# crockwell/far

Hardware: AMD Instinct MI355X
Metric: image-pairs/sec (match+solve+regress) at 640x480 (higher is better)
Workload: dtype f32

## Files before the change

### far_amd/_lib.py

```python
import ctypes
import os

from . import flags

_HERE = os.path.dirname(os.path.abspath(__file__))
LIB_PATH = flags.value('FAR_HIP_LIB') or os.path.join(_HERE, 'lib', 'libfar_hip.so')

c_p = ctypes.c_void_p
c_i = ctypes.c_int
c_f = ctypes.c_float
c_d = ctypes.c_double
c_sz = ctypes.c_size_t
c_l = ctypes.c_long
c_u32 = ctypes.c_uint32

SIGNATURES = {
    'far_abi_version': (c_i, []),
    'far_last_hip_error': (c_i, []),
    'far_set_tuning': (c_i, [c_i, c_i]),
    'far_mfma_probe_f16': (c_i, [c_i, c_i, c_i, c_p, c_p, c_p]),
    'far_dual_softmax_workspace_bytes': (c_sz, [c_i, c_i, c_i]),
    'far_dual_softmax_stats_f32': (c_i, [c_p, c_p, c_i, c_i, c_i, c_i, c_f, c_f, c_f, c_p, c_p, c_p, c_p, c_p, c_p]),
    'far_coarse_match_f32': (c_i, [c_p, c_p, c_i, c_i, c_i, c_i, c_f, c_f, c_i, c_i, c_i, c_i, c_i, c_f,
                                   c_p, c_p, c_p, c_p, c_p, c_p, c_p, c_p, c_p, c_p, c_p, c_p, c_p, c_p, c_p, c_p]),
# ... 48 lines not shown
    'far_bn_train_stats_f32': (c_i, [c_p, c_l, c_i, c_p, c_p, c_f, c_f, c_p, c_p, c_p, c_p, c_p, c_p, c_p, c_l, c_p]),
    'far_bn_train_bwd_f32': (c_i, [c_p, c_p, c_p, c_p, c_p, c_p, c_l, c_i, c_i, c_f, c_p, c_p, c_p, c_p, c_p, c_l, c_p]),
    'far_conv_packed_bytes': (c_sz, [c_i, c_i, c_i, c_i, c_i]),
    'far_conv_pack_f32': (c_i, [c_p, c_i, c_i, c_i, c_i, c_i, c_i, c_p, c_p]),
    'far_weight_scale_f32': (c_i, [c_p, c_l, c_p, c_p]),
    'far_conv_pack_view_f32': (c_i, [c_p, c_l, c_l, c_l, c_i, c_i, c_i, c_i, c_i, c_p, c_p, c_p]),
    'far_enc_layer_saved_floats': (c_l, [c_p]),
    'far_enc_layer_grads_floats': (c_l, [c_p]),
    'far_enc_layer_fwd_ws_bytes': (c_l, [c_p]),
    'far_enc_layer_bwd_ws_bytes': (c_l, [c_p]),
    'far_enc_layer_grads_offsets': (c_i, [c_p, c_p]),
    'far_enc_layer_fwd': (c_i, [c_p, c_p, c_p, c_p, c_p, c_p, c_l, c_p]),
    'far_enc_layer_bwd': (c_i, [c_p, c_p, c_p, c_p, c_p, c_p, c_p, c_l, c_p]),
    'far_stream_fork': (c_p, [c_p, c_i]),
    'far_stream_join': (c_i, [c_p, c_i]),
    'far_pack_table_bytes': (c_l, [c_i]),
    'far_pack_table_build': (c_i, [c_p, c_i, c_p, c_p]),
    'far_pack_table_run': (c_i, [c_p, c_i, c_p]),
    'far_conv_pack_view_scaled_f32': (c_i, [c_p, c_l, c_l, c_l, c_i, c_i, c_i, c_i, c_i, c_p, c_p, c_p, c_p, c_p]),
    'far_conv_pack_auto_f32': (c_i, [c_p, c_i, c_i, c_i, c_i, c_i, c_p, c_p, c_p]),
    'far_grad_scale_f32': (c_i, [c_p, c_l, c_p, c_p]),
    'far_conv_nhwc_f32': (c_i, [c_p, c_p]),
    'far_linear_kv_workspace_bytes': (c_sz, [c_l, c_i]),
    'far_linear_kv_image_bytes': (c_sz, [c_l]),
    'far_linear_kv_f16s': (c_i, [c_p, c_i, c_p, c_p, c_p, c_p]),
    'far_linear_q_apply_f16s': (c_i, [c_p, c_i, c_i, c_p, c_f, c_p]),
    'far_linear_gather_f16s': (c_i, [c_p, c_p, c_p, c_i, c_i, c_i, c_l, c_i, c_i, c_p]),
    'far_wino_packed_bytes': (c_sz, [c_i, c_i]),
    'far_wino_pack_view_scaled_f32': (c_i, [c_p, c_l, c_l, c_l, c_i, c_i, c_p, c_p, c_p, c_p, c_p]),
    'far_conv3x3_wino_f32': (c_i, [c_p, c_p]),
    'far_emm_pv_f16s_workspace_bytes': (c_sz, [c_i, c_i]),
    'far_emm_pv_f16s': (c_i, [c_p, c_p, c_p, c_p, c_i, c_i, c_i, c_f, c_i, c_l, c_l, c_i, c_p, c_p, c_p, c_p]),
    'far_emm_pv_f16': (c_i, [c_p, c_p, c_p, c_p, c_i, c_i, c_i, c_f, c_i, c_l, c_l, c_i, c_p, c_p, c_p, c_p]),
    'far_emm_pv_f16s_copy_stats': (c_i, [c_p, c_i, c_i, c_p, c_p, c_p]),
    'far_emm_bwd_workspace_bytes': (c_sz, [c_i, c_i]),
    'far_emm_bwd_f16': (c_i, [c_p, c_p, c_p, c_p, c_p, c_p, c_p, c_p, c_i, c_i, c_f, c_p, c_p, c_p, c_p]),
    'far_corr_volume_warp_workspace_bytes': (c_sz, [c_i, c_i]),
    'far_corr_volume_warp_f32': (c_i, [c_p, c_p, c_p, c_i, c_i, c_i, c_p, c_p, c_p]),
    'far_conv_wgrad_ws_bytes': (c_l, [c_i, c_i, c_i, c_i, c_i, c_i, c_i]),
    'far_conv_wgrad_f16s': (c_i, [c_p, c_p, c_i, c_i, c_i, c_i, c_i, c_i, c_i, c_i, c_p, c_p, c_l, c_p, c_p, c_p]),
    'far_stem7x7_nhwc_f32': (c_i, [c_p, c_p, c_p, c_p, c_i, c_i, c_i, c_i, c_p, c_p]),
    'far_stem7x7_wgrad_ws_bytes': (c_l, [c_i, c_i, c_i, c_i]),
    'far_stem7x7_wgrad_f32': (c_i, [c_p, c_p, c_i, c_i, c_i, c_i, c_p, c_l, c_p, c_p]),
    'far_pose_pack_f64': (c_i, [c_p] * 8 + [c_i] + [c_p] * 6 + [c_p]),
    'far_pose_features_f32': (c_i, [c_p, c_i, c_p, c_i, c_p, c_i, c_p, c_i, c_p, c_i, c_p, c_p, c_p]),
    'far_rows_linear_packed_bytes': (c_sz, [c_i, c_i]),
    'far_rows_linear_workspace_bytes': (c_sz, [c_i, c_i, c_i]),
    'far_rows_linear_pack_f32': (c_i, [c_p, c_i, c_i, c_p, c_p]),
    'far_rows_linear_f32': (c_i, [c_p, c_l, c_p, c_p, c_p, c_l, c_i, c_i, c_i, c_i, c_p, c_l, c_p, c_p]),
    'far_emm_contract_workspace_bytes': (c_sz, [c_i]),
    'far_emm_contract_f32': (c_i, [c_p, c_i, c_l, c_l, c_p, c_p, c_i, c_i, c_p, c_p, c_p]),
    'far_solver_workspace_bytes': (c_sz, [c_i, c_i, c_i, c_i]),
    'far_solver_f64': (c_i, [c_p, c_p, c_p, c_i, c_i, c_i, c_p, c_p, c_p, c_i, c_p, c_p, c_i, c_d, c_i, c_i, c_u32, c_p]
                       + [c_p] * 14 + [c_p, c_p]),
    'far_ransac_f64': (c_i, [c_p, c_p, c_p, c_i, c_i, c_i, c_p, c_p, c_p, c_i, c_d, c_i, c_i, c_u32, c_p] + [c_p] * 6 + [c_p, c_p]),
    'far_eightpoint_f64': (c_i, [c_p, c_p, c_p, c_i, c_i, c_p, c_p]),
    'far_decompose_essential_f64': (c_i, [c_p, c_l, c_p, c_p, c_p, c_p]),
    'far_build_id': (ctypes.c_char_p, []),
}



class ConvDesc(ctypes.Structure):
    _fields_ = [(n, ctypes.c_void_p) for n in ('x', 'x2', 'packed', 'scale', 'shift', 'res', 'ln_gamma', 'ln_beta',
                                               'post_res', 'up', 'y')] + \
               [('N', ctypes.c_long)] + \
# ... 68 lines not shown
```

### far_amd/csrc/emm_bilinear_f16s.hip

```cpp
#include "common.h"
#include <type_traits>

typedef float f32x4v __attribute__((ext_vector_type(4)));

namespace {

typedef _Float16 f16x8 __attribute__((ext_vector_type(8)));
typedef __attribute__((address_space(1))) const void* gptr_t;
typedef __attribute__((address_space(3))) void* lptr_t;

constexpr int D = 64;
constexpr int DV = 70;
constexpr int DVP = 96;
constexpr int KT = 64;
constexpr int CREF_ROW = 80;
constexpr float QK_PRESCALE = 16.0f;
constexpr float V_PRESCALE = 64.0f;
constexpr float NEG_HUGE = -1.0e30f;
constexpr int PAD_REF = 1 << 24;
constexpr int ROW_REF0 = -(1 << 24);

struct ZLayout {
    int heads, P, rot;
    long head_stride, prob_stride;
    __device__ __forceinline__ size_t base(long z) const {
        const long pz = z / heads;
        const int hh = (int)(z - pz * heads);
        return (size_t)hh * head_stride + (size_t)((pz + rot) % P) * prob_stride;
    }
};

__device__ __forceinline__ void split1(float x, _Float16& hi, _Float16& lo) {
    hi = (_Float16)x;
    lo = (_Float16)(x - (float)hi);
}

__global__ void k_prep_qk(const float* __restrict__ x, ZLayout lay, int Z, int N, int Np, _Float16* __restrict__ hi, _Float16* __restrict__ lo,
                          int* __restrict__ overflow) {
    const long total = (long)Z * Np * 8;
    bool bad = false;
    for (long t = (long)blockIdx.x * blockDim.x + threadIdx.x; t < total; t += (long)gridDim.x * blockDim.x) {
        const int slot = (int)(t & 7);
        const long row = t >> 3;
        const int i = (int)(row % Np);
        const long z = row / Np;
        f16x8 vh, vl;
        if (i < N) {
            const float* src = x + lay.base(z) + (size_t)i * D + slot * 8;
// ... 177 lines not shown

__global__ __launch_bounds__(256) void k_prep_v(const float* __restrict__ v, ZLayout lay, const float* __restrict__ pos,
                                               const float2* __restrict__ colstat, int Z, int N, int Np,
                                               _Float16* __restrict__ oh, _Float16* __restrict__ ol,
                                               int* __restrict__ cref) {
    __shared__ float tile[KT][DV + 3];
    const int ntile = Np / KT;
    const int z = blockIdx.x / ntile, jt = blockIdx.x - z * ntile;
    const int tid = threadIdx.x;
    for (int i = tid; i < KT * DV; i += 256) {
        const int r = i / DV, c = i - r * DV;
        const int j = jt * KT + r;
        float x = 0.f;
        if (j < N) {
            x = c < D ? v[lay.base(z) + (size_t)j * D + c] : pos[(size_t)j * 6 + (c - D)];
            const float2 cs = colstat[(size_t)z * N + j];
            x = x / (cs.y * __builtin_amdgcn_exp2f(cs.x - ceilf(cs.x))) * V_PRESCALE;
        }
        tile[r][c] = x;
    }
    if (tid < KT) {
        const int j = jt * KT + tid;
        cref[(size_t)z * Np + j] = j < N ? (int)ceilf(fminf(fmaxf(colstat[(size_t)z * N + j].x, -1.0e6f), 1.0e6f)) : PAD_REF;
    }
    __syncthreads();
    const size_t base = ((size_t)z * ntile + jt) * DVP * KT;
    for (int i = tid; i < DVP * 8; i += 256) {
        const int b = i >> 3, slot = i & 7;
        const int ct = slot >> 2, g = slot & 3;
        f16x8 vh, vl;
#pragma unroll
        for (int e = 0; e < 8; ++e) {
            const int key = 32 * ct + 16 * (g >> 1) + 4 * (g & 1) + (e < 4 ? e : e + 4);
            const float x = b < DV ? tile[key][b] : 0.f;
            _Float16 hh, ll;
            split1(x, hh, ll);
            vh[e] = hh; vl[e] = ll;
        }
        const size_t o = base + (size_t)b * KT + ((slot ^ ((b >> 1) & 7)) * 8);
        *reinterpret_cast<f16x8*>(oh + o) = vh;
        *reinterpret_cast<f16x8*>(ol + o) = vl;
    }
    __syncthreads();
    if (tid < KT) reinterpret_cast<int*>(oh + base + (size_t)CREF_ROW * KT)[tid] = cref[(size_t)z * Np + jt * KT + tid];
}

constexpr int VT_PLANE = DVP * 128;
constexpr int PV_STAGE = 2 * CT_PLANE + 2 * VT_PLANE;
template <bool MASKED>
__device__ __forceinline__ float tile_rowmax(const f32x16 (&acc)[2], float c1, int j0, int N, int h) {
    float tm = NEG_HUGE;
#pragma unroll
    for (int ct = 0; ct < 2; ++ct)
#pragma unroll
        for (int r = 0; r < 16; ++r) {
            const bool pad = MASKED && j0 + 32 * ct + mfma32_row(r, h) >= N;
            tm = fmaxf(tm, pad ? NEG_HUGE : acc[ct][r]);
        }
    return tm * c1;
}

template <bool SPLIT>
__global__ __launch_bounds__(256, 2) void k_pv(const _Float16* __restrict__ qh, const _Float16* __restrict__ ql,
                                               const _Float16* __restrict__ kh, const _Float16* __restrict__ kl,
                                               const _Float16* __restrict__ vh, const _Float16* __restrict__ vl,
                                               const int* __restrict__ cref, int Z, int N, int Np, float c1,
                                               float2* __restrict__ rowstat, float* __restrict__ T) {
    extern __shared__ __attribute__((aligned(16))) unsigned char lds_all[];
    const int tid = threadIdx.x, wave = tid >> 6, lane = tid & 63, l31 = lane & 31, h = lane >> 5;
    int z, Ib;
    tile_coords(Np / 128, Z, z, Ib);
    const int i0 = Ib * 128 + 32 * wave;
    const int irow = i0 + l31;
    RowFrags rf;
    rf.load(qh, ql, (size_t)z * Np + irow, irow, h);
    rf.arrived();

    f32x16 tacc[3];
#pragma unroll
    for (int bt = 0; bt < 3; ++bt)
#pragma unroll
        for (int r = 0; r < 16; ++r) tacc[bt][r] = 0.f;
    int R = ROW_REF0;
    float sum = 0.f, comp = 0.f;

    const int ntile = Np / KT;
    const unsigned char* vsrc_h = reinterpret_cast<const unsigned char*>(vh + (size_t)z * ntile * DVP * KT) + tid * 16;
    const unsigned char* vsrc_l = reinterpret_cast<const unsigned char*>(vl + (size_t)z * ntile * DVP * KT) + tid * 16;
    auto request = [&](int jt) {
        unsigned char* const st = lds_all + (jt & 1) * PV_STAGE;
        dma_col_tile_async(st, kh, kl, (size_t)z * Np + jt * KT, tid, wave);
        const unsigned dv = lds_addr_uniform(st + 2 * CT_PLANE + wave * 1024);
#pragma unroll
        for (int j = 0; j < 3; ++j) {
            glds16(vsrc_h + (size_t)jt * VT_PLANE + j * 4096, dv + j * 4096);
            glds16(vsrc_l + (size_t)jt * VT_PLANE + j * 4096, dv + VT_PLANE + j * 4096);
        }
    };
    request(0);
    for (int jt = 0; jt < ntile; ++jt) {
// ... 32 lines not shown
#pragma unroll
        for (int ct = 0; ct < 2; ++ct) {
#pragma unroll
            for (int u = 0; u < 2; ++u) {
                f16x8 ph, pl;
                const int4 cA = *reinterpret_cast<const int4*>(lcr + 32 * ct + 16 * u + 4 * h);
                const int4 cB = *reinterpret_cast<const int4*>(lcr + 32 * ct + 16 * u + 8 + 4 * h);
                const int cmv[8] = {cA.x, cA.y, cA.z, cA.w, cB.x, cB.y, cB.z, cB.w};
#pragma unroll
                for (int e = 0; e < 8; e += 2) {
                    const int r = 8 * u + e;
                    const f32x2 x2 = __builtin_elementwise_fma(f32x2{acc[ct][r], acc[ct][r + 1]}, f32x2{c1, c1}, f32x2{nR, nR});
                    float e0 = __builtin_amdgcn_exp2f(x2.x);
                    float e1 = __builtin_amdgcn_exp2f(x2.y);
                    if (RAGGED) {
                        if (jt * KT + 32 * ct + mfma32_row(r, h) >= N) e0 = 0.f;
                        if (jt * KT + 32 * ct + mfma32_row(r + 1, h) >= N) e1 = 0.f;
                    }
                    t2 += f32x2{e0, e1};
                    const f32x2 p2 = f32x2{e0, e1} * f32x2{ldexpf(e0, R - cmv[e] + 15), ldexpf(e1, R - cmv[e + 1] + 15)};
                    f16x2 h2, l2;
                    if (SPLIT) split2(p2, h2, l2);
                    else { h2 = __builtin_convertvector(p2, f16x2); l2 = h2; }
                    ph[e] = h2.x; ph[e + 1] = h2.y;
                    pl[e] = l2.x; pl[e + 1] = l2.y;
                }
                const int slot = 4 * ct + 2 * u + h;
#pragma unroll
                for (int bt = 0; bt < 3; ++bt) {
                    const int b = 32 * bt + l31;
                    const int off = b * 128 + ((slot ^ ((b >> 1) & 7)) * 16);
                    const f16x8 bh = *reinterpret_cast<const f16x8*>(ldv + off);
                    tacc[bt] = __builtin_amdgcn_mfma_f32_32x32x16_f16(ph, bh, tacc[bt], 0, 0, 0);
                    if (SPLIT) {
                        const f16x8 bl = *reinterpret_cast<const f16x8*>(ldv + VT_PLANE + off);
                        tacc[bt] = __builtin_amdgcn_mfma_f32_32x32x16_f16(ph, bl, tacc[bt], 0, 0, 0);
                        tacc[bt] = __builtin_amdgcn_mfma_f32_32x32x16_f16(pl, bh, tacc[bt], 0, 0, 0);
                    }
                }
            }
        }
        };
        if (ragged) pv_tile(std::true_type{});
        else pv_tile(std::false_type{});
        const float y = (t2.x + t2.y) - comp;
        const float ns = sum + y;
        comp = (ns - sum) - y;
        sum = ns;
    }
    sum -= comp;
    const float rsum = sum + shfl_xor_f(sum, 32);
    if (h == 0 && irow < N) rowstat[(size_t)z * N + irow] = make_float2((float)R, rsum);
    const float oscale = (3.0517578125e-05f / V_PRESCALE) / rsum;
#pragma unroll
    for (int bt = 0; bt < 3; ++bt) {
        const int b = 32 * bt + l31;
#pragma unroll
        for (int r = 0; r < 16; ++r) {
            const int rr = mfma32_row(r, h);
            const float sc = __shfl(oscale, rr, 64);
            const int i = i0 + rr;
            if (b < DV && i < N) T[((size_t)z * N + i) * DV + b] = tacc[bt][r] * sc;
        }
    }
}

inline size_t align256(size_t x) { return (x + 255) & ~(size_t)255; }
struct EmmWs {
    _Float16 *qh, *ql, *kh, *kl, *vh, *vl;
    float2 *rowstat, *colstat;
    int* cref;
    size_t bytes;
};
inline EmmWs carve(void* base, int Z, int N) {
    const int Np = (N + 127) / 128 * 128;
    unsigned char* p = (unsigned char*)base;
    size_t o = 0;
    auto take = [&](size_t n) { unsigned char* r = p ? p + o : nullptr; o += align256(n); return r; };
    EmmWs w;
    const size_t qk = (size_t)Z * Np * D * 2, vt = (size_t)Z * (Np / KT) * DVP * KT * 2, st = (size_t)Z * N * 8;
    w.qh = (_Float16*)take(qk); w.ql = (_Float16*)take(qk); w.kh = (_Float16*)take(qk); w.kl = (_Float16*)take(qk);
    w.vh = (_Float16*)take(vt); w.vl = (_Float16*)take(vt);
    w.rowstat = (float2*)take(st); w.colstat = (float2*)take(st);
    w.cref = (int*)take((size_t)Z * Np * 4);
    w.bytes = o;
    return w;
}

}

extern "C" {

size_t far_emm_pv_f16s_workspace_bytes(int Z, int N) {
    if (Z <= 0 || N <= 0) return 0;
    return carve(nullptr, Z, N).bytes;
}

}

template <bool SPLIT>
static int emm_pv_launch(const float* q, const float* k, const float* v, const float* pos, int Z, int N, int Dh, float scale,
                         int heads, long head_stride, long prob_stride, int q_rot, void* ws, float* T_out, int* overflow,
                         hipStream_t stream) {
    far_clear_errors();
    if (!q || !k || !v || !pos || !ws || !T_out || Z <= 0 || N <= 0 || Dh != D || heads < 1 || Z % heads || q_rot < 0 ||
        q_rot >= Z / heads)
        return FAR_EINVAL;
    const ZLayout lay{heads, Z / heads, 0, head_stride, prob_stride};
    const ZLayout layq{heads, Z / heads, q_rot, head_stride, prob_stride};
    const int Np = (N + 127) / 128 * 128;
    const EmmWs w = carve(ws, Z, N);
    const float c1 = scale * 1.44269504088896341f / (QK_PRESCALE * QK_PRESCALE);
    const unsigned gprep = (unsigned)(((long)Z * Np * 8 + 255) / 256 < 65536L * 4 ? ((long)Z * Np * 8 + 255) / 256 : 65536L * 4);
    hipLaunchKernelGGL(k_prep_qk, dim3(gprep), dim3(256), 0, stream, q, layq, Z, N, Np, w.qh, w.ql, overflow);
    hipLaunchKernelGGL(k_prep_qk, dim3(gprep), dim3(256), 0, stream, k, lay, Z, N, Np, w.kh, w.kl, overflow);
    const dim3 grid((unsigned)(Np / 128) * Z);
    const dim3 gstat((unsigned)(Np / 128) * Z);
    hipLaunchKernelGGL(k_rowstats<SPLIT>, gstat, dim3(256), 0, stream, w.kh, w.kl, w.qh, w.ql, Z, N, Np, c1, w.colstat);
    hipLaunchKernelGGL(k_prep_v, dim3((unsigned)(Np / KT) * Z), dim3(256), 0, stream, v, lay, pos, w.colstat, Z, N, Np, w.vh, w.vl, w.cref);
    bool cfg_failed = false;
    FAR_ONCE_PER_DEVICE(cfg_failed = hipFuncSetAttribute((const void*)k_pv<SPLIT>, hipFuncAttributeMaxDynamicSharedMemorySize, 2 * PV_STAGE) != hipSuccess);
    if (cfg_failed) return far_check_launch();
    hipLaunchKernelGGL(k_pv<SPLIT>, grid, dim3(256), 2 * PV_STAGE, stream, w.qh, w.ql, w.kh, w.kl, w.vh, w.vl, w.cref, Z, N, Np, c1,
                       w.rowstat, T_out);
    return far_check_launch();
}

extern "C" {

int far_emm_pv_f16s(const float* q, const float* k, const float* v, const float* pos, int Z, int N, int Dh, float scale,
                    int heads, long head_stride, long prob_stride, int q_rot, void* ws, float* T_out, int* overflow,
                    hipStream_t stream) {
    return emm_pv_launch<true>(q, k, v, pos, Z, N, Dh, scale, heads, head_stride, prob_stride, q_rot, ws, T_out, overflow, stream);
}

int far_emm_pv_f16(const float* q, const float* k, const float* v, const float* pos, int Z, int N, int Dh, float scale,
                   int heads, long head_stride, long prob_stride, int q_rot, void* ws, float* T_out, int* overflow,
                   hipStream_t stream) {
    return emm_pv_launch<false>(q, k, v, pos, Z, N, Dh, scale, heads, head_stride, prob_stride, q_rot, ws, T_out, overflow, stream);
}

int far_emm_pv_f16s_copy_stats(const void* ws, int Z, int N, float* rowstat_out, float* colstat_out, hipStream_t stream) {
    far_clear_errors();
    if (!ws || !rowstat_out || !colstat_out || Z <= 0 || N <= 0) return FAR_EINVAL;
    const EmmWs w = carve(const_cast<void*>(ws), Z, N);
    hipMemcpyAsync(rowstat_out, w.rowstat, (size_t)Z * N * 8, hipMemcpyDeviceToDevice, stream);
    hipMemcpyAsync(colstat_out, w.colstat, (size_t)Z * N * 8, hipMemcpyDeviceToDevice, stream);
    return far_check_launch();
}

}
```

### far_amd/flags.py

```python
import os
from collections import namedtuple

Switch = namedtuple('Switch', 'env module attr off_value neutral scope doc')
SWITCHES = [
    Switch('FAR_NO_WINO', 'far_amd.ops', 'USE_WINO', False, 'parity', 'inference',
           'stride-1 3x3 convolutions on K9 (direct implicit GEMM) instead of K17 (Winograd F(2x2,3x3)); same operator, other summation'),
    Switch('FAR_NO_PAD', 'far_amd.loftr.backbone', 'PAD_CHANNELS', False, 'bitwise', 'inference',
           'the 196-channel backbone maps stored with 196 channels instead of 208 (zero weights for the extra ones: exact zeros)'),
    Switch('FAR_NO_PREFETCH', 'far_amd.loftr.model:LoFTR', 'head_prefetch', False, 'bitwise', 'inference',
           "the head's feature stage computed inside forward_rt_prediction instead of enqueued behind K1"),
    Switch('FAR_NO_SIDE_STREAM', 'far_amd.loftr.model:LoFTR', 'head_side_stream', False, 'bitwise', 'inference',
           "the head's feature stage on the step's own stream behind K1 (rounds 2-5) instead of on a second stream next to K1 and the fine level"),
    Switch('FAR_FPN_STREAM', 'far_amd.loftr.model:LoFTR', 'fpn_side_stream', True, 'bitwise', 'inference',
           "OPT-IN (1 switches it ON; default off): the FPN's fine branch on a side stream next to the coarse transformer and K1 (-0.6 ms per 32 "
           "pairs; off by default because the roofline launch -- K17 208 -> 208 @ 240x320 -- then shares the GPU and its in-step duration "
           "in a kernel trace is no longer its own)"),
    Switch('FAR_NO_GATHER_FUSE', 'far_amd.loftr.stages:FinePreprocess', 'fused_gather', False, 'bitwise', 'inference',
           'FinePreprocess.merge_feat on a materialised window tensor (K3 gather + K9) instead of K9 reading through the match indices'),
    Switch('FAR_NO_KV', 'far_amd.loftr.transformer:LoFTREncoderLayer', 'fused_kv', False, 'parity', 'inference',
           "k, v projections + K5's first half as separate launches instead of K9's k|v epilogue (the K'^T V sum changes order)"),
    Switch('FAR_NO_QAPPLY', 'far_amd.loftr.transformer:LoFTREncoderLayer', 'fused_apply', False, 'parity', 'inference',
           "q projection + K5's second half as separate launches instead of K9's attention-apply epilogue (q no longer stays in split operands)"),
    Switch('FAR_NO_STACK', 'far_amd.loftr.transformer:LocalFeatureTransformer', 'stack_self', False, 'bitwise', 'inference',
           "the two 'self' calls of an encoder layer on the two images separately instead of one call on both"),
    Switch('FAR_NO_BN', 'far_amd.ops', 'USE_HIP_BATCHNORM_TRAIN', False, 'parity', 'training',
           'training-mode BatchNorm on nn.BatchNorm2d + torch activations instead of K19 (tests/test_train_kernels_gpu.py holds K19 to the module)'),
]

ENV_ONLY = {
    'FAR_HIP_LIB': ('load', 'path of another build of libfar_hip.so (tools/ab_build.py: same-box A/B against a git revision); skips the build-id check'),
    'FAR_TUNING': ('load', 'comma-separated key=value pairs handed to far_set_tuning at load time, e.g. FAR_TUNING="10=1,8=1" (keys below)'),
    'FAR_SKIP_ASM_CHECK': ('build', "1: far_amd/build.py does not scan the generated code (K9's asm pixel loads; the LDS-DMA ring rule of every kernel with global_load_lds; the half-register writes of the asm fp16 split) after recompiling"),
    'FAR_EXTRA_HIPCC_FLAGS': ('build', 'extra hipcc flags of an experiment build (-DFAR_WINO_EXP=..., tools/wino_exp.sh); part of the build id'),
    'FAR_COMMIT': ('tools', 'commit stamp tools/collect_profiles.sh / tools/step_floors.py write into the profile files'),
    'FAR_C3_PY_NODE': ('bench', "bench.py --workload c3: the encoder layer's autograd node driven from Python instead of far_enc_layer_fwd / _bwd"),
    'FAR_C3_NO_OVERLAP': ('bench', 'bench.py --workload c3: the layer node without side streams'),
    'FAR_C3_PER_OP': ('bench', 'bench.py --workload c3: one autograd node per operator instead of per layer'),
    'FAR_TORCH_ADAMW': ('bench', 'bench.py --workload c3: torch.optim.AdamW instead of K20'),
    'FAR_CUDNN_BENCHMARK': ('bench', 'bench.py: torch.backends.cudnn.benchmark for the vendor comparison legs'),
}

Tuning = namedtuple('Tuning', 'key default values neutral doc')
TUNING = [
    Tuning(0, 3, (0, 1, 2, 4, 7), 'bitwise', 'bit mask of exact-f32 kernels that stagger wave-slot priorities: 1 k_stats, 2 k_match, 4 k_emm_pv'),
    Tuning(1, 0, (1,), 'parity', 'K1 exact-f32 variant: the other tile shape (another summation order of the row statistics)'),
    Tuning(2, 0, (1,), 'bitwise', 'conf_matrix writer variant A (store pattern)'),
    Tuning(3, 0, (1,), 'bitwise', 'conf_matrix writer variant B (store pattern)'),
    Tuning(4, 0, (1,), 'bitwise', 'K9 without the seven-tile mode / K5 windows on the generic path'),
    Tuning(5, 0, (1, 2, 4), 'bitwise', 'K5 apply: tiles per unit'),
    Tuning(6, 0, (64, 256), 'parity', "K5: tokens per K'^T V chunk (another partial-sum grouping)"),
    Tuning(7, 0, (1,), 'bitwise', 'K9 Linear launches always on full-height tiles'),
    Tuning(8, 0, (1,), 'bitwise', 'K17 splits its operands with the five-instruction split2 instead of v_fma_mix (same values)'),
    Tuning(9, 0, (1,), 'bitwise', 'K17 runs a short last channel block on the full body'),
    Tuning(10, 0, (1,), 'bitwise', "K1's match pass without the tile prescreen"),
    Tuning(11, 0, (1, 2), 'bitwise', "K14's pipeline: 0 = 4 waves / 3 slots / counted waits, two workgroups per CU; 1 = 8 waves / 4 slots / counted, one per CU (round 5's form); 2 = 4 waves / 3 slots / vmcnt(0) per phase (fallback without a wait table)"),
    Tuning(12, 0, (1,), 'parity', "K10's inference form on the exact-f32 matrix instruction instead of split fp16"),
    Tuning(15, 0, (1,), 'bitwise', 'K17: 1 = the multiplying wave group does NOT raise its issue priority (the round-4 kernel)'),
    Tuning(13, 0, (1,), 'bitwise', "K9's FPN-merge epilogue in its generic form everywhere"),
]


def off(env):
    if env not in {s.env for s in SWITCHES}:
        raise KeyError(f'{env} is not a registered far_amd switch (far_amd/flags.py)')
    return os.environ.get(env, '0') not in ('', '0')


def value(env, default=None):
    if env not in ENV_ONLY:
        raise KeyError(f'{env} is not a registered far_amd environment variable (far_amd/flags.py)')
    return os.environ.get(env, default)


def known():
    return {s.env for s in SWITCHES} | set(ENV_ONLY)


def unknown_in_environment():
    skip = ('FAR_WINO_', 'FAR_K9_')
    return sorted(k for k in os.environ if k.startswith('FAR_') and k not in known() and not k.startswith(skip))


def target(sw):
    import importlib
    mod, _, cls = sw.module.partition(':')
    obj = importlib.import_module(mod)
    return (getattr(obj, cls) if cls else obj), sw.attr
```

### far_amd/loftr/transformer.py

```python
import copy
import os
from functools import partial

import torch
import torch.nn as nn

from .. import _vendor as ag
from .. import flags, ops
from ..pose6d import pose_mean_6d, pose_std_6d


class LinearAttention(nn.Module):

    def __init__(self, eps=1e-6, use_num_corres=False):
        super().__init__()
        self.eps = eps
        self.use_num_corres = use_num_corres

    def forward(self, queries, keys, values, q_mask=None, kv_mask=None, loftr_preds=None):
        N, L, H, D = queries.shape
        S = keys.shape[1]
        if ag.needs_grad(queries, keys, values):
            if queries.is_cuda and D in (16, 32):
                return ops.linear_attention_train(queries.reshape(N, L, H * D), keys.reshape(N, S, H * D),
# ... 237 lines not shown
    return torch.stack([p3 * p3, p4 * p4, p3 * p4, p3, p4, torch.ones_like(p3)], dim=1).contiguous()


def positional_table_vit(h=24, w=24, intrinsics=None):
    if h != w:
        raise ValueError('the reference indexes this table with k*w + j, which covers the grid only when h == w (24 x 24)')
    ys = torch.linspace(-1, 1, steps=h)
    xs = torch.linspace(-1, 1, steps=w)
    if intrinsics is None:
        p3 = ys.repeat(w)
        p4 = xs.repeat_interleave(h)
    else:
        fx, fy, cx, cy = (torch.tensor(float(v), dtype=torch.float32) for v in intrinsics)
        hpix, wpix = cy * 2, cx * 2
        K = torch.zeros(3, 3)
        K[0, 0] = (fx / wpix) * 2
        K[1, 1] = (fy / hpix) * 2
        K[0, 2] = (cx / wpix) * 2 - 1
        K[1, 2] = (cy / hpix) * 2 - 1
        K[2, 2] = 1
        Kinv = torch.inverse(K)
        gx, gy = torch.meshgrid(xs, ys, indexing='ij')
        pts = torch.stack([gx.reshape(-1), gy.reshape(-1), torch.ones(h * w)], 0)
        wv = Kinv @ pts
        p4 = wv[0] / wv[2]
        p3 = wv[1] / wv[2]
    return torch.stack([p3 * p3, p4 * p4, p3 * p4, p3, p4, torch.ones_like(p3)], dim=1).contiguous()


class CrossAttention(nn.Module):
    hip_training = True
    plain16 = False
    exact_f32 = False

    def __init__(self, dim, num_heads=8, qkv_bias=False, attn_drop=0., proj_drop=0., pos=None):
        super().__init__()
        self.num_heads = num_heads
        self.scale = (dim // num_heads) ** -0.5
        self.qkv = nn.Linear(dim, dim * 3, bias=qkv_bias)
        self.proj_fundamental = nn.Linear(dim + 6 * num_heads, dim)
        self.register_buffer('pos6', positional_table() if pos is None else pos.detach().float().contiguous(), persistent=False)

    def forward(self, x1, x2, intrinsics=None, loftr_preds=None, inv_loftr_preds=None):
        B, N, C = x1.shape
        if not x1.is_cuda:
            ag.require('CrossAttention on CPU tensors')
        h, d = self.num_heads, C // self.num_heads
        if self.pos6.shape[0] != N:
            raise ValueError(f'the positional table of this CrossAttention has {self.pos6.shape[0]} rows (mp3d: the 60x80 coarse grid, '
                             f'transformer.py:194), got N={N} tokens')
        if ag.needs_grad(x1, x2, self.qkv.weight) or not x1.is_cuda:
            qkv = self.qkv(torch.stack([x1, x2], 0)).reshape(2, B, N, 3, h, d).permute(3, 0, 1, 4, 2, 5).contiguous()
            q, k, v = qkv[0], qkv[1], qkv[2]
            qq = torch.stack([q[1], q[0]], 0).reshape(2 * B * h, N, d)
            kk, vv = k.reshape(2 * B * h, N, d), v.reshape(2 * B * h, N, d)
            if x1.is_cuda and d == 64 and self.hip_training:
                F = ops.emm_bilinear_train(qq, kk, vv, self.pos6, self.scale)
            else:
                F = ag.require('CrossAttention on CPU tensors or with hip_training = False').bilinear_attention(qq, kk, vv, self.pos6, self.scale)
        else:
            pk = self.__dict__.setdefault('_packs', ops.PackCache())
            ts = [self.qkv.weight] + ([self.qkv.bias] if self.qkv.bias is not None else [])
            pc = pk.get(('qkv', self.plain16), ts, lambda: ops.PackedConv(self.qkv.weight, None, self.qkv.bias, split=not self.plain16))
            adjacent = (x1.is_contiguous() and x2.is_contiguous() and x1.shape == x2.shape and
                        x1.untyped_storage().data_ptr() == x2.untyped_storage().data_ptr() and
                        x2.storage_offset() == x1.storage_offset() + x1.numel())
            x12 = torch.as_strided(x1, (2, B, N, C), (B * N * C, N * C, C, 1)) if adjacent else torch.stack([x1, x2], 0)
            planes = ops.linear_f16s(x12.reshape(2 * B, N, C), pc, out_planes=3 * h)
            if self.exact_f32:
                P = planes.view(3, h, 2, B, N, d).permute(0, 2, 3, 1, 4, 5)
                qq = torch.stack([P[0, 1], P[0, 0]], 0).reshape(2 * B * h, N, d).contiguous()
                F, _ = ops.emm_bilinear(qq, P[1].reshape(2 * B * h, N, d).contiguous(), P[2].reshape(2 * B * h, N, d).contiguous(),
                                        self.pos6, self.scale, exact_f32=True)
            else:
                F, _ = ops.emm_bilinear_planes(planes, self.pos6, self.scale, B, plain16=self.plain16)
        F = F.view(2, B, h, d + 6, d + 6)
        f1 = F[0].reshape(B, C + 6 * h, (C + 6 * h) // h).transpose(-2, -1)
        f2 = F[1].reshape(B, C + 6 * h, (C + 6 * h) // h).transpose(-2, -1)
        if ag.needs_grad(f1, self.proj_fundamental.weight) or not f1.is_cuda:
            f2 = self.proj_fundamental(f2)
            f1 = self.proj_fundamental(f1)
        else:
            pk = self.__dict__.setdefault('_packs', ops.PackCache())
            pw, pb = self.proj_fundamental.weight, self.proj_fundamental.bias
            pad = (-pw.shape[1]) % 4
            pp = pk.get('proj', [pw, pb], lambda: ops.PackedConv(nn.functional.pad(pw.detach(), (0, pad)) if pad else pw, None, pb))
            f12 = torch.stack([f1, f2], 0)
            f12 = ops.linear_f16s(nn.functional.pad(f12, (0, pad)) if pad else f12.contiguous(), pp)
            f1, f2 = f12[0], f12[1]
        return f2, f1


def _init_vit(m):
    if isinstance(m, nn.Linear):
        nn.init.trunc_normal_(m.weight, std=.02)
        if m.bias is not None:
            nn.init.zeros_(m.bias)
    elif isinstance(m, nn.LayerNorm):
        nn.init.zeros_(m.bias)
        nn.init.ones_(m.weight)


class CrossBlock(nn.Module):
    def __init__(self, dim, num_heads, mlp_ratio=4., qkv_bias=False, drop=0., attn_drop=0., drop_path=0.,
                 act_layer=nn.GELU, norm_layer=nn.LayerNorm, use_pos_embedding=False, distilled=False, pos=None):
        super().__init__()
        self.norm1 = norm_layer(dim)
        self.cross_attn = CrossAttention(dim, num_heads=num_heads, qkv_bias=qkv_bias, pos=pos)
# ... 181 lines not shown
```

### far_amd/ops/head.py

```python
import ctypes
import os
import threading

import torch

from .. import _lib, flags
from ._base import _p, _stream, _ws, overflow_flag
from .coarse import dual_softmax_stats


def emm_bilinear(q, k, v, pos, scale, exact_f32=False, plain16=False):
    lib = _lib.load()
    Z, N, D = q.shape
    T = torch.empty(Z, N, 70, dtype=torch.float32, device=q.device)
    if exact_f32:
        rowstat, colstat = dual_softmax_stats(q, k, 1.0, 1.0, scale)
        rc = lib.far_emm_pv_f32(_p(q, torch.float32), _p(k, torch.float32), _p(v, torch.float32), _p(pos, torch.float32),
                                Z, N, D, float(scale), _p(rowstat), _p(colstat), _p(T), _stream())
        _lib.check(rc, 'far_emm_pv_f32')
    else:
        ws = _ws(lib.far_emm_pv_f16s_workspace_bytes(Z, N), q.device)
        name = 'far_emm_pv_f16' if plain16 else 'far_emm_pv_f16s'
        rc = getattr(lib, name)(_p(q, torch.float32), _p(k, torch.float32), _p(v, torch.float32), _p(pos, torch.float32),
                                Z, N, D, float(scale), 1, 0, N * D, 0, _p(ws), _p(T), _p(overflow_flag(T.device)), _stream())
# ... 32 lines not shown
    def backward(ctx, dF):
        lib = _lib.load()
        qc, kc, vc, posc, T, rs, cs = ctx.saved_tensors
        Z, N, D = qc.shape
        dF = dF.float().contiguous()
        vt = torch.cat([vc, posc.unsqueeze(0).expand(Z, -1, -1)], dim=2).contiguous()
        Tp = _emm_pv(kc, qc, vc, posc, ctx.scale)
        A = torch.bmm(vt, dF)
        Bm = torch.bmm(vt, dF.transpose(1, 2))
        dvt = torch.bmm(T, dF.transpose(1, 2)) + torch.bmm(Tp, dF)
        u = (A * T).sum(-1)
        vw = (Bm * Tp).sum(-1)
        tiny = 1e-30
        bound = (1.0 / rs[..., 1].amin()) * (2.0 * A.norm(dim=-1).amax() * vt.norm(dim=-1).amax() + u.abs().amax()) \
            + (1.0 / cs[..., 1].amin()) * vw.abs().amax()
        alpha = torch.minimum(2.0 ** 11 / A.abs().amax().clamp_min(tiny), 2.0 ** 14 / bound.clamp_min(tiny))
        alpha = torch.exp2(torch.floor(torch.log2(alpha)))
        u = (u * alpha).contiguous()
        vw = (vw * alpha).contiguous()
        A = (A * alpha).contiguous()
        dq, dk = torch.empty_like(qc), torch.empty_like(kc)
        ws = _ws(lib.far_emm_bwd_workspace_bytes(Z, N), qc.device)
        rc = lib.far_emm_bwd_f16(_p(qc), _p(kc), _p(vt, torch.float32), _p(A, torch.float32), _p(u, torch.float32),
                                 _p(vw, torch.float32), _p(rs), _p(cs), Z, N, ctx.scale, _p(dq), _p(dk), _p(ws), _stream())
        _lib.check(rc, 'far_emm_bwd_f16')
        inv = 1.0 / alpha
        return dq * inv, dk * inv, dvt[:, :, :D].contiguous(), None, None

def emm_bilinear_train(q, k, v, pos, scale):
    if not q.is_cuda:
        raise _lib.FarHipError('far_amd ops need tensors on the GPU (no CPU fallback exists)')
    return _EmmBilinearFn.apply(q, k, v, pos, scale)

def emm_bilinear_planes(qkv, pos, scale, B, plain16=False):
    lib = _lib.load()
    P12, P, N, D = qkv.shape
    h = P12 // 3
    Z = P * h
    T = torch.empty(Z, N, 70, dtype=torch.float32, device=qkv.device)
    ws = _ws(lib.far_emm_pv_f16s_workspace_bytes(Z, N), qkv.device)
    base = qkv.data_ptr()
    plane = P * N * D * 4
    name = 'far_emm_pv_f16' if plain16 else 'far_emm_pv_f16s'
    rc = getattr(lib, name)(ctypes.c_void_p(base), ctypes.c_void_p(base + h * plane), ctypes.c_void_p(base + 2 * h * plane),
                            _p(pos, torch.float32), Z, N, D, float(scale), h, P * N * D, N * D, B, _p(ws), _p(T), _p(overflow_flag(T.device)), _stream())
    _lib.check(rc, name)
    return emm_contract(ctypes.c_void_p(base + 2 * h * plane), h, P * N * D, N * D, pos, T), T

def solve_pose_batch(kpts0, kpts1, offsets_host, K0, K1, inl_th, many_thr, priorRT=None, pcl=None,
                     prior_lambda=0.3, H=2048, seed=0, samples=None, debug=False, minimal=8):
    lib = _lib.load()
    dev = K0.device
    offs = torch.as_tensor(offsets_host, dtype=torch.int32)
    B = offs.numel() - 1
    Mtot = int(offs[-1])
    Mmax = int((offs[1:] - offs[:-1]).max()) if B > 0 else 0
    offs_d = offs.pin_memory().to(dev, non_blocking=True)
    P = 0 if pcl is None else int(pcl.shape[0])
    ws = _ws(lib.far_solver_workspace_bytes(B, Mtot, H, P), dev)
    f64, i32 = torch.float64, torch.int32
    out = {
        'R': torch.empty(B, 3, 3, dtype=f64, device=dev), 't': torch.empty(B, 3, dtype=f64, device=dev),
        'E': torch.empty(B, 3, 3, dtype=f64, device=dev), 'mask': torch.empty(Mtot, dtype=torch.uint8, device=dev),
        'status': torch.empty(B, dtype=i32, device=dev), 'num_after': torch.empty(B, dtype=i32, device=dev),
        'tight': torch.empty(B, dtype=i32, device=dev), 'ultra': torch.empty(B, dtype=i32, device=dev),
        'n_cheir': torch.empty(B, dtype=i32, device=dev), 'best': torch.empty(B, dtype=i32, device=dev),
    }
    dbg = {}
    if debug:
        dbg = {'F_all': torch.empty(B, H, 3, 3, dtype=f64, device=dev), 'count_all': torch.empty(B, H, dtype=i32, device=dev),
               'score_all': torch.empty(B, H, dtype=f64, device=dev),
               'samples': torch.full((B, H, 8) if minimal == 8 else (B, max(H // 10, 1), 5), -1, dtype=i32, device=dev)}
    rc = lib.far_solver_f64(
        _p(kpts0, torch.float32) if Mtot else ctypes.c_void_p(0), _p(kpts1, torch.float32) if Mtot else ctypes.c_void_p(0),
        _p(offs_d), B, Mtot, Mmax, _p(K0.contiguous(), f64), _p(K1.contiguous(), f64), _p(inl_th, f64), int(bool(many_thr)),
# ... 119 lines not shown
```

### include/far_hip.h

```cpp
#ifndef FAR_HIP_H
#define FAR_HIP_H

#include <stddef.h>
#include <stdint.h>

#ifdef __cplusplus
extern "C" {
#endif

typedef struct ihipStream_t* far_stream_t;

int far_abi_version(void);
const char* far_build_id(void);
int far_last_hip_error(void);
int far_set_tuning(int key, int value);

void* far_stream_fork(far_stream_t main, int i);
int far_stream_join(far_stream_t main, int i);

int far_mfma_probe_f16(int mode, int iters, int rounds, float* sink, double* flops_out, far_stream_t stream);


size_t far_dual_softmax_workspace_bytes(int Z, int L, int S);

// ... 41 lines not shown
                                   int64_t* b_ids, int64_t* i_ids, int64_t* j_ids, float* mconf,
                                   float* mkpts0_c, float* mkpts1_c, int* counts_out, int* total_out,
                                   void* ws, int* overflow, far_stream_t stream);

size_t far_coarse_train_workspace_bytes(int Z, int L, int S, int C);
int far_coarse_pos_conf_f16s(const float* f0, const float* f1, int Z, int L, int S, int C, float temperature,
                             const int64_t* pb, const int64_t* pi, const int64_t* pj, int M, float* p_out, void* ws,
                             int* overflow, far_stream_t stream);
int far_coarse_pos_conf_bwd_f16(const float* f0, const float* f1, int Z, int L, int S, int C, float temperature,
                                const int64_t* pb, const int64_t* pi, const int64_t* pj, int M, const float* w,
                                float* df0, float* df1, void* ws, far_stream_t stream);

size_t far_sinkhorn_pos_conf_workspace_bytes(int Z, int L, int S, int C, int iters);
int far_sinkhorn_pos_conf_f16s(const float* f0, const float* f1, int Z, int L, int S, int C, const float* bin_score, int iters,
                               const uint8_t* mask0, const uint8_t* mask1, const int64_t* pb, const int64_t* pi, const int64_t* pj,
                               int M, float* conf_pos, float* conf_bin0, float* conf_bin1, void* ws, int* overflow,
                               far_stream_t stream);
int far_sinkhorn_pos_conf_bwd_f16(const float* f0, const float* f1, int Z, int L, int S, int C, const float* bin_score, int iters,
                                  const uint8_t* mask0, const uint8_t* mask1, const int64_t* pb, const int64_t* pi, const int64_t* pj,
                                  int M, const float* w_pos, const float* w_bin0, const float* w_bin1, float* df0, float* df1,
                                  float* dbin, void* ws, far_stream_t stream);


int far_emm_pv_f32(const float* q, const float* k, const float* v, const float* pos, int Z, int N, int D,
                   float scale, const float* rowstat, const float* colstat, float* T_out, far_stream_t stream);

size_t far_emm_pv_f16s_workspace_bytes(int Z, int N);
int far_emm_pv_f16s(const float* q, const float* k, const float* v, const float* pos, int Z, int N, int D, float scale,
                    int heads, long head_stride, long prob_stride, int q_rot, void* ws, float* T_out, int* overflow,
                    far_stream_t stream);
int far_emm_pv_f16(const float* q, const float* k, const float* v, const float* pos, int Z, int N, int D, float scale,
                   int heads, long head_stride, long prob_stride, int q_rot, void* ws, float* T_out, int* overflow,
                   far_stream_t stream);
int far_emm_pv_f16s_copy_stats(const void* ws, int Z, int N, float* rowstat_out, float* colstat_out, far_stream_t stream);

size_t far_emm_bwd_workspace_bytes(int Z, int N);
int far_emm_bwd_f16(const float* q, const float* k, const float* vt, const float* A, const float* u, const float* vw,
                    const float* rowstat, const float* colstat, int Z, int N, float scale, float* dq, float* dk,
                    void* ws, far_stream_t stream);


int far_fine_gather_f32(const float* feat, long sn, long sc, long sh, long sw, int C, int Hf, int Wf,
                        const int64_t* b_ids, const int64_t* cell_ids, int wc, int W, int stride, int M,
                        float* out, far_stream_t stream);

int far_fine_scatter_f32(const float* dout, long sn, long sc, long sh, long sw, int C, int Hf, int Wf,
                         const int64_t* b_ids, const int64_t* cell_ids, int wc, int W, int stride, int M,
                         float* dfeat, far_stream_t stream);
int far_fine_scatter_det_f32(const float* dout, long sn, long sc, long sh, long sw, int C, int Hf, int Wf, const int64_t* order,
                             const int* start, int Z, int hc, int wc, int W, int stride, int M, float* dfeat, far_stream_t stream);
int far_fine_expect_f32(const float* feat0, const float* feat1, int M, int W, int C, const float* mkpts1_c,
                        float win_scale, const float* scale1, const int64_t* b_ids, float* expec_f,
                        float* mkpts1_f, far_stream_t stream);

size_t far_linear_attention_workspace_bytes(int N, int S, int H, int D);

int far_linear_attention_f32(const float* q, const float* k, const float* v, int N, int L, int S, int H, int D,
                             const uint8_t* q_mask, const uint8_t* kv_mask, float eps, float* out, void* ws,
                             far_stream_t stream);

int far_linear_attention_apply_f32(const float* q, const float* kv, int N, int L, int S, int H, const uint8_t* q_mask, float eps,
                                   float* out, far_stream_t stream);

size_t far_full_attention_workspace_bytes(int N, int L, int S, int H, int D);
int far_full_attention_f16s(const float* q, const float* k, const float* v, int N, int L, int S, int H, int D,
                            const uint8_t* q_mask, const uint8_t* kv_mask, int act_exp, float* out, void* ws,
// ... 193 lines not shown
```

Baseline: 375.9.

## Fuse the K2 contraction into k_pv's epilogue with per-tile partials

```diff
diff --git a/far_amd/_lib.py b/far_amd/_lib.py
--- a/far_amd/_lib.py
+++ b/far_amd/_lib.py
@@ -104,6 +104,8 @@
     'far_emm_pv_f16s_workspace_bytes': (c_sz, [c_i, c_i]),
     'far_emm_pv_f16s': (c_i, [c_p, c_p, c_p, c_p, c_i, c_i, c_i, c_f, c_i, c_l, c_l, c_i, c_p, c_p, c_p, c_p]),
     'far_emm_pv_f16': (c_i, [c_p, c_p, c_p, c_p, c_i, c_i, c_i, c_f, c_i, c_l, c_l, c_i, c_p, c_p, c_p, c_p]),
+    'far_emm_pv_contract_f16s_workspace_bytes': (c_sz, [c_i, c_i]),
+    'far_emm_pv_contract_f16s': (c_i, [c_p, c_p, c_p, c_p, c_i, c_i, c_i, c_f, c_i, c_l, c_l, c_i, c_p, c_p, c_p, c_p]),
     'far_emm_pv_f16s_copy_stats': (c_i, [c_p, c_i, c_i, c_p, c_p, c_p]),
     'far_emm_bwd_workspace_bytes': (c_sz, [c_i, c_i]),
     'far_emm_bwd_f16': (c_i, [c_p, c_p, c_p, c_p, c_p, c_p, c_p, c_p, c_i, c_i, c_f, c_p, c_p, c_p, c_p]),
diff --git a/far_amd/csrc/emm_bilinear_f16s.hip b/far_amd/csrc/emm_bilinear_f16s.hip
--- a/far_amd/csrc/emm_bilinear_f16s.hip
+++ b/far_amd/csrc/emm_bilinear_f16s.hip
@@ -14,6 +14,7 @@
 constexpr int DVP = 96;
 constexpr int KT = 64;
 constexpr int CREF_ROW = 80;
+constexpr int POS_LO_ROW = 70;
 constexpr float QK_PRESCALE = 16.0f;
 constexpr float V_PRESCALE = 64.0f;
 constexpr float NEG_HUGE = -1.0e30f;
@@ -257,10 +258,10 @@
 #pragma unroll
         for (int e = 0; e < 8; ++e) {
             const int key = 32 * ct + 16 * (g >> 1) + 4 * (g & 1) + (e < 4 ? e : e + 4);
-            const float x = b < DV ? tile[key][b] : 0.f;
+            const float x = b < DV ? tile[key][b] : b < POS_LO_ROW + 6 ? tile[key][b - 6] : 0.f;
             _Float16 hh, ll;
             split1(x, hh, ll);
-            vh[e] = hh; vl[e] = ll;
+            vh[e] = b < DV ? hh : ll; vl[e] = b < DV ? ll : (_Float16)0.f;
         }
         const size_t o = base + (size_t)b * KT + ((slot ^ ((b >> 1) & 7)) * 8);
         *reinterpret_cast<f16x8*>(oh + o) = vh;
@@ -285,12 +286,22 @@
     return tm * c1;
 }
 
-template <bool SPLIT>
+struct ContractArgs {
+    const float* v;
+    ZLayout lay;
+    const float* pos;
+    float* part;
+};
+constexpr int RSTR = 72;
+
+template <bool SPLIT, int FUSED = 0>
 __global__ __launch_bounds__(256, 2) void k_pv(const _Float16* __restrict__ qh, const _Float16* __restrict__ ql,
                                                const _Float16* __restrict__ kh, const _Float16* __restrict__ kl,
                                                const _Float16* __restrict__ vh, const _Float16* __restrict__ vl,
                                                const int* __restrict__ cref, int Z, int N, int Np, float c1,
-                                               float2* __restrict__ rowstat, float* __restrict__ T) {
+                                               float2* __restrict__ rowstat, float* __restrict__ T, ContractArgs ca) {
+    static_assert(FUSED == 0 || SPLIT, "the fused contraction exists for split operands only");
+    static_assert(4 * DV * RSTR * 4 <= 2 * PV_STAGE, "the four waves' partials must fit the tile stages");
     extern __shared__ __attribute__((aligned(16))) unsigned char lds_all[];
     const int tid = threadIdx.x, wave = tid >> 6, lane = tid & 63, l31 = lane & 31, h = lane >> 5;
     int z, Ib;
@@ -389,7 +400,9 @@
                     const int off = b * 128 + ((slot ^ ((b >> 1) & 7)) * 16);
                     const f16x8 bh = *reinterpret_cast<const f16x8*>(ldv + off);
                     tacc[bt] = __builtin_amdgcn_mfma_f32_32x32x16_f16(ph, bh, tacc[bt], 0, 0, 0);
-                    if (SPLIT) {
+                    if (SPLIT && FUSED == 2 && bt == 2) {
+                        tacc[bt] = __builtin_amdgcn_mfma_f32_32x32x16_f16(pl, bh, tacc[bt], 0, 0, 0);
+                    } else if (SPLIT) {
                         const f16x8 bl = *reinterpret_cast<const f16x8*>(ldv + VT_PLANE + off);
                         tacc[bt] = __builtin_amdgcn_mfma_f32_32x32x16_f16(ph, bl, tacc[bt], 0, 0, 0);
                         tacc[bt] = __builtin_amdgcn_mfma_f32_32x32x16_f16(pl, bh, tacc[bt], 0, 0, 0);
@@ -407,8 +420,102 @@
     }
     sum -= comp;
     const float rsum = sum + shfl_xor_f(sum, 32);
-    if (h == 0 && irow < N) rowstat[(size_t)z * N + irow] = make_float2((float)R, rsum);
+    int lc = l31;
+    if constexpr (FUSED != 0) asm volatile("" : "+v"(lc));
+    const int irow_st = i0 + lc;
+    if (h == 0 && irow_st < N) rowstat[(size_t)z * N + irow_st] = make_float2((float)R, rsum);
     const float oscale = (3.0517578125e-05f / V_PRESCALE) / rsum;
+    if constexpr (FUSED != 0) {
+        const float* const vz = ca.v + ca.lay.base(z);
+        float av[3][2][8];
+#pragma unroll
+        for (int at = 0; at < 3; ++at)
+#pragma unroll
+            for (int u = 0; u < 2; ++u)
+#pragma unroll
+                for (int e = 0; e < 8; ++e) {
+                    const int i = i0 + mfma32_row(8 * u + e, h);
+                    const int ic = i < N ? i : N - 1;
+                    const float x = at < 2 ? vz[(size_t)ic * D + 32 * at + lc] : ca.pos[(size_t)ic * (DV - D) + (lc < DV - D ? lc : 0)];
+                    av[at][u][e] = (i < N && (at < 2 || lc < DV - D)) ? x : 0.f;
+                }
+        __syncthreads();
+        float amax = 0.f;
+#pragma unroll
+        for (int bt = 0; bt < 3; ++bt) {
+            const int b = 32 * bt + l31;
+#pragma unroll
+            for (int r = 0; r < 16; ++r) {
+                const int rr = mfma32_row(r, h);
+                const float sc = __shfl(oscale, rr, 64);
+                float t = tacc[bt][r];
+                if (FUSED == 2 && bt == 2) t += __shfl_down(t, POS_LO_ROW - D, 64);
+                t = (b < DV && i0 + rr < N) ? t * sc : 0.f;
+                tacc[bt][r] = t;
+                amax = fmaxf(amax, fabsf(t));
+            }
+        }
+#pragma unroll
+        for (int m = 32; m; m >>= 1) amax = fmaxf(amax, shfl_xor_f(amax, m));
+        int ex = 0;
+        (void)frexpf(amax, &ex);
+        int sT = 15 - ex;
+        sT = sT < -100 ? -100 : sT > 100 ? 100 : sT;
+        f16x8 th[3][2], tl[3][2];
+#pragma unroll
+        for (int bt = 0; bt < 3; ++bt)
+#pragma unroll
+            for (int u = 0; u < 2; ++u)
+#pragma unroll
+                for (int e = 0; e < 8; e += 2) {
+                    f16x2 h2, l2;
+                    split2(f32x2{ldexpf(tacc[bt][8 * u + e], sT), ldexpf(tacc[bt][8 * u + e + 1], sT)}, h2, l2);
+                    th[bt][u][e] = h2.x; th[bt][u][e + 1] = h2.y;
+                    tl[bt][u][e] = l2.x; tl[bt][u][e + 1] = l2.y;
+                }
+        const float unscale = ldexpf(1.0f, -(sT + 4));
+        float* const red = reinterpret_cast<float*>(lds_all);
+#pragma unroll
+        for (int at = 0; at < 3; ++at) {
+            f32x16 facc[3];
+#pragma unroll
+            for (int bt = 0; bt < 3; ++bt)
+#pragma unroll
+                for (int r = 0; r < 16; ++r) facc[bt][r] = 0.f;
+#pragma unroll
+            for (int u = 0; u < 2; ++u) {
+                f16x8 ah, al;
+#pragma unroll
+                for (int e = 0; e < 8; e += 2) {
+                    f16x2 h2, l2;
+                    split2(f32x2{av[at][u][e] * QK_PRESCALE, av[at][u][e + 1] * QK_PRESCALE}, h2, l2);
+                    ah[e] = h2.x; ah[e + 1] = h2.y;
+                    al[e] = l2.x; al[e + 1] = l2.y;
+                }
+#pragma unroll
+                for (int bt = 0; bt < 3; ++bt) {
+                    facc[bt] = __builtin_amdgcn_mfma_f32_32x32x16_f16(ah, th[bt][u], facc[bt], 0, 0, 0);
+                    facc[bt] = __builtin_amdgcn_mfma_f32_32x32x16_f16(ah, tl[bt][u], facc[bt], 0, 0, 0);
+                    facc[bt] = __builtin_amdgcn_mfma_f32_32x32x16_f16(al, th[bt][u], facc[bt], 0, 0, 0);
+                }
+            }
+#pragma unroll
+            for (int bt = 0; bt < 3; ++bt)
+#pragma unroll
+                for (int r = 0; r < 16; ++r) {
+                    const int a = 32 * at + mfma32_row(r, h), b = 32 * bt + l31;
+                    if (a < DV && b < DV) red[(wave * DV + a) * RSTR + b] = facc[bt][r] * unscale;
+                }
+        }
+        __syncthreads();
+        float* const slot = ca.part + ((size_t)z * (Np / 128) + Ib) * (DV * DV);
+        for (int idx = tid; idx < DV * DV; idx += 256) {
+            const int a = idx / DV, b = idx - a * DV;
+            const float* const p = red + a * RSTR + b;
+            slot[idx] = ((p[0] + p[DV * RSTR]) + p[2 * DV * RSTR]) + p[3 * DV * RSTR];
+        }
+        return;
+    }
 #pragma unroll
     for (int bt = 0; bt < 3; ++bt) {
         const int b = 32 * bt + l31;
@@ -443,6 +550,17 @@
     w.bytes = o;
     return w;
 }
+inline size_t contract_part_bytes(int Z, int N) { return align256((size_t)Z * ((N + 127) / 128) * DV * DV * 4); }
+
+__global__ void k_contract_sum(const float* __restrict__ part, int nblk, long total, float* __restrict__ F) {
+    const long i = (long)blockIdx.x * blockDim.x + threadIdx.x;
+    if (i >= total) return;
+    const long z = i / (DV * DV);
+    const float* p = part + (size_t)z * (nblk - 1) * (DV * DV) + i;
+    float v = p[0];
+    for (int s = 1; s < nblk; ++s) v += p[(size_t)s * (DV * DV)];
+    F[i] = v;
+}
 
 }
 
@@ -453,14 +571,19 @@
     return carve(nullptr, Z, N).bytes;
 }
 
-}
-
-template <bool SPLIT>
+size_t far_emm_pv_contract_f16s_workspace_bytes(int Z, int N) {
+    if (Z <= 0 || N <= 0) return 0;
+    return carve(nullptr, Z, N).bytes + contract_part_bytes(Z, N);
+}
+
+}
+
+template <bool SPLIT, int FUSED = 0>
 static int emm_pv_launch(const float* q, const float* k, const float* v, const float* pos, int Z, int N, int Dh, float scale,
-                         int heads, long head_stride, long prob_stride, int q_rot, void* ws, float* T_out, int* overflow,
+                         int heads, long head_stride, long prob_stride, int q_rot, void* ws, float* out, int* overflow,
                          hipStream_t stream) {
     far_clear_errors();
-    if (!q || !k || !v || !pos || !ws || !T_out || Z <= 0 || N <= 0 || Dh != D || heads < 1 || Z % heads || q_rot < 0 ||
+    if (!q || !k || !v || !pos || !ws || !out || Z <= 0 || N <= 0 || Dh != D || heads < 1 || Z % heads || q_rot < 0 ||
         q_rot >= Z / heads)
         return FAR_EINVAL;
     const ZLayout lay{heads, Z / heads, 0, head_stride, prob_stride};
@@ -476,10 +599,15 @@
     hipLaunchKernelGGL(k_rowstats<SPLIT>, gstat, dim3(256), 0, stream, w.kh, w.kl, w.qh, w.ql, Z, N, Np, c1, w.colstat);
     hipLaunchKernelGGL(k_prep_v, dim3((unsigned)(Np / KT) * Z), dim3(256), 0, stream, v, lay, pos, w.colstat, Z, N, Np, w.vh, w.vl, w.cref);
     bool cfg_failed = false;
-    FAR_ONCE_PER_DEVICE(cfg_failed = hipFuncSetAttribute((const void*)k_pv<SPLIT>, hipFuncAttributeMaxDynamicSharedMemorySize, 2 * PV_STAGE) != hipSuccess);
+    FAR_ONCE_PER_DEVICE(cfg_failed = hipFuncSetAttribute((const void*)k_pv<SPLIT, FUSED>, hipFuncAttributeMaxDynamicSharedMemorySize, 2 * PV_STAGE) != hipSuccess);
     if (cfg_failed) return far_check_launch();
-    hipLaunchKernelGGL(k_pv<SPLIT>, grid, dim3(256), 2 * PV_STAGE, stream, w.qh, w.ql, w.kh, w.kl, w.vh, w.vl, w.cref, Z, N, Np, c1,
-                       w.rowstat, T_out);
+    float* const part = FUSED ? reinterpret_cast<float*>((unsigned char*)ws + w.bytes) : nullptr;
+    hipLaunchKernelGGL((k_pv<SPLIT, FUSED>), grid, dim3(256), 2 * PV_STAGE, stream, w.qh, w.ql, w.kh, w.kl, w.vh, w.vl, w.cref, Z, N, Np, c1,
+                       w.rowstat, FUSED ? nullptr : out, ContractArgs{v, lay, pos, part});
+    if (FUSED) {
+        const long total = (long)Z * DV * DV;
+        hipLaunchKernelGGL(k_contract_sum, dim3((unsigned)((total + 255) / 256)), dim3(256), 0, stream, part, Np / 128, total, out);
+    }
     return far_check_launch();
 }
 
@@ -489,6 +617,14 @@
                     int heads, long head_stride, long prob_stride, int q_rot, void* ws, float* T_out, int* overflow,
                     hipStream_t stream) {
     return emm_pv_launch<true>(q, k, v, pos, Z, N, Dh, scale, heads, head_stride, prob_stride, q_rot, ws, T_out, overflow, stream);
+}
+
+int far_emm_pv_contract_f16s(const float* q, const float* k, const float* v, const float* pos, int Z, int N, int Dh, float scale,
+                             int heads, long head_stride, long prob_stride, int q_rot, void* ws, float* F_out, int* overflow,
+                             hipStream_t stream) {
+    if (far_get_tuning(14) == 0)
+        return emm_pv_launch<true, 2>(q, k, v, pos, Z, N, Dh, scale, heads, head_stride, prob_stride, q_rot, ws, F_out, overflow, stream);
+    return emm_pv_launch<true, 1>(q, k, v, pos, Z, N, Dh, scale, heads, head_stride, prob_stride, q_rot, ws, F_out, overflow, stream);
 }
 
 int far_emm_pv_f16(const float* q, const float* k, const float* v, const float* pos, int Z, int N, int Dh, float scale,
diff --git a/far_amd/flags.py b/far_amd/flags.py
--- a/far_amd/flags.py
+++ b/far_amd/flags.py
@@ -23,6 +23,9 @@
            "q projection + K5's second half as separate launches instead of K9's attention-apply epilogue (q no longer stays in split operands)"),
     Switch('FAR_NO_STACK', 'far_amd.loftr.transformer:LocalFeatureTransformer', 'stack_self', False, 'bitwise', 'inference',
            "the two 'self' calls of an encoder layer on the two images separately instead of one call on both"),
+    Switch('FAR_NO_K2_CONTRACT', 'far_amd.loftr.transformer:CrossAttention', 'fused_contract', False, 'parity', 'inference',
+           "K2 as far_emm_pv_f16s + far_emm_contract_f32 through a (Z, N, 70) tensor instead of the contraction in k_pv's epilogue "
+           '(far_emm_pv_contract_f16s: F on split operands, the pos tile in two products, another summation order)'),
     Switch('FAR_NO_BN', 'far_amd.ops', 'USE_HIP_BATCHNORM_TRAIN', False, 'parity', 'training',
            'training-mode BatchNorm on nn.BatchNorm2d + torch activations instead of K19 (tests/test_train_kernels_gpu.py holds K19 to the module)'),
 ]
@@ -55,6 +58,7 @@
     Tuning(10, 0, (1,), 'bitwise', "K1's match pass without the tile prescreen"),
     Tuning(11, 0, (1, 2), 'bitwise', "K14's pipeline: 0 = 4 waves / 3 slots / counted waits, two workgroups per CU; 1 = 8 waves / 4 slots / counted, one per CU (round 5's form); 2 = 4 waves / 3 slots / vmcnt(0) per phase (fallback without a wait table)"),
     Tuning(12, 0, (1,), 'parity', "K10's inference form on the exact-f32 matrix instruction instead of split fp16"),
+    Tuning(14, 0, (1,), 'parity', "K2's fused form (far_emm_pv_contract_f16s): 1 = the pos tile of P v~ as three products from both planes instead of two from the hi plane"),
     Tuning(15, 0, (1,), 'bitwise', 'K17: 1 = the multiplying wave group does NOT raise its issue priority (the round-4 kernel)'),
     Tuning(13, 0, (1,), 'bitwise', "K9's FPN-merge epilogue in its generic form everywhere"),
 ]
diff --git a/far_amd/loftr/transformer.py b/far_amd/loftr/transformer.py
--- a/far_amd/loftr/transformer.py
+++ b/far_amd/loftr/transformer.py
@@ -293,6 +293,7 @@
     hip_training = True
     plain16 = False
     exact_f32 = False
+    fused_contract = not flags.off('FAR_NO_K2_CONTRACT')
 
     def __init__(self, dim, num_heads=8, qkv_bias=False, attn_drop=0., proj_drop=0., pos=None):
         super().__init__()
@@ -334,7 +335,8 @@
                 F, _ = ops.emm_bilinear(qq, P[1].reshape(2 * B * h, N, d).contiguous(), P[2].reshape(2 * B * h, N, d).contiguous(),
                                         self.pos6, self.scale, exact_f32=True)
             else:
-                F, _ = ops.emm_bilinear_planes(planes, self.pos6, self.scale, B, plain16=self.plain16)
+                F, _ = ops.emm_bilinear_planes(planes, self.pos6, self.scale, B, plain16=self.plain16,
+                                               need_T=self.plain16 or not self.fused_contract)
         F = F.view(2, B, h, d + 6, d + 6)
         f1 = F[0].reshape(B, C + 6 * h, (C + 6 * h) // h).transpose(-2, -1)
         f2 = F[1].reshape(B, C + 6 * h, (C + 6 * h) // h).transpose(-2, -1)
diff --git a/far_amd/ops/head.py b/far_amd/ops/head.py
--- a/far_amd/ops/head.py
+++ b/far_amd/ops/head.py
@@ -88,15 +88,33 @@
         raise _lib.FarHipError('far_amd ops need tensors on the GPU (no CPU fallback exists)')
     return _EmmBilinearFn.apply(q, k, v, pos, scale)
 
-def emm_bilinear_planes(qkv, pos, scale, B, plain16=False):
+def emm_bilinear_fused(q, k, v, pos, scale):
+    lib = _lib.load()
+    Z, N, D = q.shape
+    F = torch.empty(Z, 70, 70, dtype=torch.float32, device=q.device)
+    ws = _ws(lib.far_emm_pv_contract_f16s_workspace_bytes(Z, N), q.device)
+    rc = lib.far_emm_pv_contract_f16s(_p(q, torch.float32), _p(k, torch.float32), _p(v, torch.float32), _p(pos, torch.float32),
+                                      Z, N, D, float(scale), 1, 0, N * D, 0, _p(ws), _p(F), _p(overflow_flag(F.device)), _stream())
+    _lib.check(rc, 'far_emm_pv_contract_f16s')
+    return F
+
+def emm_bilinear_planes(qkv, pos, scale, B, plain16=False, need_T=True):
     lib = _lib.load()
     P12, P, N, D = qkv.shape
     h = P12 // 3
     Z = P * h
+    base = qkv.data_ptr()
+    plane = P * N * D * 4
+    if not need_T and not plain16:
+        F = torch.empty(Z, 70, 70, dtype=torch.float32, device=qkv.device)
+        ws = _ws(lib.far_emm_pv_contract_f16s_workspace_bytes(Z, N), qkv.device)
+        rc = lib.far_emm_pv_contract_f16s(ctypes.c_void_p(base), ctypes.c_void_p(base + h * plane), ctypes.c_void_p(base + 2 * h * plane),
+                                          _p(pos, torch.float32), Z, N, D, float(scale), h, P * N * D, N * D, B, _p(ws), _p(F),
+                                          _p(overflow_flag(F.device)), _stream())
+        _lib.check(rc, 'far_emm_pv_contract_f16s')
+        return F, None
     T = torch.empty(Z, N, 70, dtype=torch.float32, device=qkv.device)
     ws = _ws(lib.far_emm_pv_f16s_workspace_bytes(Z, N), qkv.device)
-    base = qkv.data_ptr()
-    plane = P * N * D * 4
     name = 'far_emm_pv_f16' if plain16 else 'far_emm_pv_f16s'
     rc = getattr(lib, name)(ctypes.c_void_p(base), ctypes.c_void_p(base + h * plane), ctypes.c_void_p(base + 2 * h * plane),
                             _p(pos, torch.float32), Z, N, D, float(scale), h, P * N * D, N * D, B, _p(ws), _p(T), _p(overflow_flag(T.device)), _stream())
diff --git a/include/far_hip.h b/include/far_hip.h
--- a/include/far_hip.h
+++ b/include/far_hip.h
@@ -97,6 +97,10 @@
 int far_emm_pv_f16(const float* q, const float* k, const float* v, const float* pos, int Z, int N, int D, float scale,
                    int heads, long head_stride, long prob_stride, int q_rot, void* ws, float* T_out, int* overflow,
                    far_stream_t stream);
+size_t far_emm_pv_contract_f16s_workspace_bytes(int Z, int N);
+int far_emm_pv_contract_f16s(const float* q, const float* k, const float* v, const float* pos, int Z, int N, int D, float scale,
+                             int heads, long head_stride, long prob_stride, int q_rot, void* ws, float* F_out, int* overflow,
+                             far_stream_t stream);
 int far_emm_pv_f16s_copy_stats(const void* ws, int Z, int N, float* rowstat_out, float* colstat_out, far_stream_t stream);
 
 size_t far_emm_bwd_workspace_bytes(int Z, int N);
```

Result: no change. 376.3 (median of 4 runs) (+0.1%).
